# amirkdv/biseqt

Hardware: AMD Instinct MI355X
Metric: GCUPS (DP cell updates/s) banded local align (higher is better)
Workload: dtype i16

## Files before the change

### biseqt_amd/csrc/pw_wave.h

```cpp
#ifndef PW_WAVE_H
#define PW_WAVE_H

#ifndef PW_FN
#error "PW_FN must be defined by the includer"
#endif

#include "pw_types.h"

namespace pw {

template <typename T> struct ScoreTraits;
template <> struct ScoreTraits<int32_t> {
  static constexpr bool is_int = true;
  PW_FN static int32_t neg() { return -(1 << 28); }
  PW_FN static int32_t zero_blk() { return 0; }
  PW_FN static int32_t max2(int32_t a, int32_t b) { return a > b ? a : b; }
  PW_FN static int32_t gap_offer(bool kept, int32_t go, int32_t A) { return kept ? A : A + go; }
};
template <> struct ScoreTraits<double> {
  static constexpr bool is_int = false;
  PW_FN static double neg() { return -1.0e300; }
  PW_FN static double zero_blk() { return -0.0; }
  PW_FN static double max2(double a, double b) { return __builtin_fmax(a, b); }
  union D2I_ { double d; int32_t i[2]; };
// ... 273 lines not shown
    const int wo = (xfeed_o + 8 * b) >> 2, wm = (yfeed_m + 8 * b) >> 2;
    fo_n0 = P::const_dword(oseq, pw_clampi(wo, 0, owlast)); fo_n1 = P::const_dword(oseq, pw_clampi(wo + 1, 0, owlast));
    fo_n2 = P::const_dword(oseq, pw_clampi(wo + 2, 0, owlast));
    fm_n0 = P::const_dword(mseq, pw_clampi(wm, 0, mwlast)); fm_n1 = P::const_dword(mseq, pw_clampi(wm + 1, 0, mwlast));
    fm_n2 = P::const_dword(mseq, pw_clampi(wm + 2, 0, mwlast));
  }
  PW_FN void feed_commit(int b) {
    const int ro = (xfeed_o + 8 * b) & 3, rm = (yfeed_m + 8 * b) & 3;
    fo_lo = funnel(fo_n1, fo_n0, ro); fo_hi = funnel(fo_n2, fo_n1, ro);
    fm_lo = funnel(fm_n1, fm_n0, rm); fm_hi = funnel(fm_n2, fm_n1, rm);
  }

  template <bool RAMP>
  PW_FN void block(int b) {
    if (RAMP) {
#pragma unroll 1
      for (int k = 0; k < 8; k++) iteration<true>(8 * b + k, k);
    } else {
#pragma unroll
      for (int k = 0; k < 8; k++) iteration<false>(8 * b + k, k);
    }
  }

  PW_FN void store_masks(int b) {
    if (lane >= 0 && lane * BK < ndiag && P::central()) {
      uint32_t* dst = a.masks + pd.mask_off;
#pragma unroll
      for (int j = 0; j < BK; j++) dst[mask_word_index(BK, pd.nl, b, lane, j)] = m[j];
    }
  }

  PW_FN void init(int it0 = 0) {
    lane = P::lane();
    X = pd.X; Y = pd.Y; ndiag = pd.ndiag;
    oseq = a.arena + pd.o_off; mseq = a.arena + pd.m_off;
    olast = X > 0 ? X - 1 : 0; mlast = Y > 0 ? Y - 1 : 0;
    owlast = olast >> 2; mwlast = mlast >> 2;
    njl = lane < 0 ? 0 : ndiag - lane * BK;
    uin_next = Tr::neg();
    const int e = (pd.s0 + pd.dmin) >> 1;
    const int f = (pd.s0 - pd.dmin) >> 1;
    xbase = e + it0 + lane * R;
    ybase = f + it0 - lane * R;
    xfeed_o = e + P::nlanes() * R - 1;
    yfeed_m = f - P::lane0() * R;
#pragma unroll
    for (int j = 0; j < BK; j++) {
      H[j] = Tr::neg(); U[j] = Tr::neg(); L[j] = Tr::neg();
      best[j] = Tr::neg(); bestT[j] = 0; m[j] = 0;
      blkL[j] = (lane * BK + j == ndiag) ? Tr::neg() : Tr::zero_blk();
    }
#pragma unroll
    for (int i = 0; i < R; i++) {
      ow[i] = (uint32_t)oseq[pw_clampi(xbase + i - 1, 0, olast)] * osc();
      mw[i] = (uint32_t)mseq[pw_clampi(ybase - i - 1, 0, mlast)] * msc();
    }
    if (AHEAD) {
#pragma unroll
      for (int i = 0; i < (AHEAD ? R : 1); i++) sE[i] = subst(ow[i], mw[i]);
    }
  }

  PW_FN void run() {
    init();
    feed_issue(0);
    for (int b = 0; b < pd.nblocks; b++) {
      feed_commit(b);
      if (b + 1 < pd.nblocks) feed_issue(b + 1);
      if (b >= pd.steady_b0 && b < pd.steady_b1) block<false>(b);
      else block<true>(b);
      store_masks(b);
    }
    finish();
  }

  PW_FN void run_tile() {
    const int bb0 = a.tile_b0, bb1 = a.tile_b0 + a.tile_nb, pitch = a.st_pitch;
    lane = P::lane();
    ndiag = pd.ndiag;
    int w4[4] = {-0x7fffffff, -0x7fffffff, -0x7fffffff, -0x7fffffff};
#pragma unroll
    for (int j = 0; j < BK; j++) {
      const int dd = lane * BK + j;
      if (lane >= 0 && dd < ndiag) {
        const int d = pd.dmin + dd;
        const int tf = (d < 0 ? -d : d) - pd.s0;
        const int tl = tf + 2 * ((d > 0 ? 0 : d) + (pd.X - d > pd.Y ? pd.Y : pd.X - d));
        w4[0] = -tf > w4[0] ? -tf : w4[0]; w4[1] = tf > w4[1] ? tf : w4[1];
        w4[2] = -tl > w4[2] ? -tl : w4[2]; w4[3] = tl > w4[3] ? tl : w4[3];
      }
    }
    P::wg_max4(w4);
    const int tfmin = -w4[0], tfmax = w4[1], tlmin = -w4[2], tlmax = w4[3];
    int bA = tfmin >> 4, bB = tlmax >> 4;
    if (w4[1] == -0x7fffffff) { bA = 1; bB = 0; }
    bA = bA < bb0 ? bb0 : bA; bB = bB > bb1 - 1 ? bb1 - 1 : bB;
    if (bA > bB) {
      if (P::central()) {
#pragma unroll
        for (int j = 0; j < BK; j++) {
          const int dd = lane * BK + j;
          if (lane >= 0 && dd < ndiag) {
#pragma unroll
            for (int r = 0; r < 5; r++)
              a.st_out[r * pitch + dd] = bb0 > 0 ? a.st_in[r * pitch + dd] : (r == 4 ? T(0) : Tr::neg());
          }
        }
      }
      return;
    }
    init(8 * bA);
    if (bb0 > 0) {
#pragma unroll
      for (int j = 0; j < BK; j++) {
        const int dd = lane * BK + j;
        if (lane >= 0 && dd < ndiag) {
          H[j] = a.st_in[dd]; U[j] = a.st_in[pitch + dd]; L[j] = a.st_in[2 * pitch + dd];
          best[j] = a.st_in[3 * pitch + dd]; bestT[j] = (int32_t)a.st_in[4 * pitch + dd];
        }
      }
      uint32_t none = 0;
      uin_next = U[BK - 1];
      xshift_pair<P, false>(uin_next, Tr::neg(), none, 0u, 1);
    }
    feed_issue(bA);
    for (int b = bA; b <= bB; b++) {
      feed_commit(b);
      if (b < bB) feed_issue(b + 1);
      if (16 * b > tfmax && 16 * b + 15 <= tlmin) block<false>(b);
      else block<true>(b);
      store_masks(b);
    }
    if (P::central()) {
#pragma unroll
      for (int j = 0; j < BK; j++) {
        const int dd = lane * BK + j;
        if (lane >= 0 && dd < ndiag) {
          a.st_out[dd] = H[j]; a.st_out[pitch + dd] = U[j]; a.st_out[2 * pitch + dd] = L[j];
          a.st_out[3 * pitch + dd] = best[j]; a.st_out[4 * pitch + dd] = (T)bestT[j];
        }
      }
    }
  }

  PW_FN void finish() {
    const int endrule = a.endrule;
    T cs = Tr::neg(); uint64_t ck = ~(uint64_t)0; int cx = -1, cy = -1; bool have = false;
#pragma unroll
    for (int j = 0; j < BK; j++) {
      const int dd = lane * BK + j;
      const int d = pd.dmin + dd;
      const bool inband = dd < ndiag;
      const bool ends_right = d < X - Y;
      const int lx = ends_right ? d + Y : X, ly = ends_right ? Y : X - d;
      T s; uint64_t k; int x, y; bool ok = inband;
      if (endrule == END_CORNER) {
        ok = ok && (d == X - Y); s = H[j]; k = 0; x = X; y = Y;
      } else if (endrule == END_STD_OVERLAP) {
        s = H[j]; x = lx; y = ly; k = ends_right ? (uint64_t)(uint32_t)lx : (uint64_t)(uint32_t)(X + ly);
      } else if (endrule == END_BANDED_OVERLAP) {
        s = H[j]; x = lx; y = ly; k = (uint64_t)(uint32_t)dd;
      } else {
        const int tfirst = (d < 0 ? -d : d) - pd.s0;
        const int aa = (bestT[j] - tfirst) >> 1;
        s = best[j]; x = aa + (d > 0 ? d : 0); y = aa - (d < 0 ? d : 0);
        if (endrule == END_STD_LOCAL) k = (uint64_t)(uint32_t)x * (uint64_t)(uint32_t)(Y + 1) + (uint64_t)(uint32_t)y;
        else k = ((uint64_t)(uint32_t)dd << 32) | (uint64_t)(uint32_t)aa;
      }
      const bool better = ok && (!have || s > cs || (s == cs && k < ck));
      if (better) { cs = s; ck = k; cx = x; cy = y; have = true; }
    }
    int hv = have ? 1 : 0;
#pragma unroll
    for (int off = 32; off >= 1; off >>= 1) {
      const T os = xshfl_xor<P>(cs, off);
      const uint64_t ok_ = xshfl_xor<P>(ck, off);
      const int ox = P::shfl_xor(cx, off), oy = P::shfl_xor(cy, off), oh = P::shfl_xor(hv, off);
      const bool take = oh && (!hv || os > cs || (os == cs && ok_ < ck));
      if (take) { cs = os; ck = ok_; cx = ox; cy = oy; hv = 1; }
    }
    if (P::nwaves() > 1) {
      T bs = cs; uint64_t bk_ = ck; int bx = cx, by = cy, bh = 0;
      for (int wv = 0; wv < P::nwaves(); wv++) {
        const T os = xwave_bcast<P>(cs, wv);
        const uint64_t ok_ = xwave_bcast<P>(ck, wv);
        const int ox = P::wave_bcast(cx, wv), oy = P::wave_bcast(cy, wv), oh = P::wave_bcast(hv, wv);
        const bool take = oh && (!bh || os > bs || (os == bs && ok_ < bk_));
        if (take) { bs = os; bk_ = ok_; bx = ox; by = oy; bh = 1; }
      }
      cs = bs; ck = bk_; cx = bx; cy = by; hv = bh;
    }
    if (lane == 0) {
      Result r;
      r.score = (double)cs * a.score_mul;
      r.opt_i = a.banded ? cx - cy - pd.dmin : cx;
      r.opt_j = a.banded ? (cx < cy ? cx : cy) : cy;
      r.origin_idx = 0; r.mutant_idx = 0; r.tx_len = 0; r.status = 0;
      if (!hv || (endrule == END_STD_LOCAL && !(cs > T(0)))) { r.opt_i = -1; r.opt_j = -1; r.score = 0.0; }
      a.results[pair_slot] = r;
    }
  }
  int pair_slot;
};

struct __attribute__((aligned(8))) U4 { uint32_t x, y, z, w; };
struct __attribute__((packed)) PackedU64 { uint64_t v; };
struct __attribute__((packed)) PackedU32 { uint32_t v; };

namespace pk {
#if defined(__HIP_DEVICE_COMPILE__)
typedef short s2_t __attribute__((ext_vector_type(2)));
typedef unsigned short u2_t __attribute__((ext_vector_type(2)));
PW_FN s2_t as_s2(uint32_t v) { return __builtin_bit_cast(s2_t, v); }
PW_FN u2_t as_u2(uint32_t v) { return __builtin_bit_cast(u2_t, v); }
PW_FN uint32_t add(uint32_t a, uint32_t b) { return __builtin_bit_cast(uint32_t, (u2_t)(as_u2(a) + as_u2(b))); }
PW_FN uint32_t sub(uint32_t a, uint32_t b) { return __builtin_bit_cast(uint32_t, (u2_t)(as_u2(a) - as_u2(b))); }
PW_FN uint32_t subsat(uint32_t a, uint32_t b) { return __builtin_bit_cast(uint32_t, __builtin_elementwise_sub_sat(as_u2(a), as_u2(b))); }
PW_FN uint32_t max(uint32_t a, uint32_t b) { return __builtin_bit_cast(uint32_t, __builtin_elementwise_max(as_s2(a), as_s2(b))); }
PW_FN uint32_t minu(uint32_t a, uint32_t b) { return __builtin_bit_cast(uint32_t, __builtin_elementwise_min(as_u2(a), as_u2(b))); }
PW_FN uint32_t maxu(uint32_t a, uint32_t b) { return __builtin_bit_cast(uint32_t, __builtin_elementwise_max(as_u2(a), as_u2(b))); }
PW_FN uint32_t shru(uint32_t a, uint32_t sh) { return __builtin_bit_cast(uint32_t, (u2_t)(as_u2(a) >> as_u2(sh))); }
PW_FN uint32_t mad(uint32_t a, uint32_t b, uint32_t c) { return __builtin_bit_cast(uint32_t, (u2_t)(as_u2(a) * as_u2(b) + as_u2(c))); }
PW_FN uint32_t mins(uint32_t a, uint32_t b) { return __builtin_bit_cast(uint32_t, __builtin_elementwise_min(as_s2(a), as_s2(b))); }
PW_FN uint32_t align16(uint32_t hi, uint32_t lo) { return __builtin_amdgcn_alignbit(hi, lo, 16); }
PW_FN uint32_t sign(uint32_t a, uint32_t sh15) { return __builtin_bit_cast(uint32_t, (s2_t)(as_s2(a) >> as_s2(sh15))); }
PW_FN uint32_t opaque(uint32_t v) { asm volatile("" : "+v"(v)); return v; }
PW_FN uint32_t opaque_su(uint32_t v) { asm volatile("" : "+s"(v)); return v; }
PW_FN uint8_t* opaque_s(uint8_t* v) { asm volatile("" : "+s"(v)); return v; }
PW_FN void store_global(uint8_t* base, uint32_t off, const U4& v) {
  typedef __attribute__((address_space(1))) uint8_t gbyte_t;
  typedef __attribute__((address_space(1))) U4 gu4_t;
  *(gu4_t*)((gbyte_t*)base + off) = v;
}
PW_FN uint32_t perm(uint32_t a, uint32_t b, uint32_t sel) { return __builtin_amdgcn_perm(a, b, sel); }
#else
PW_FN uint32_t mk(uint32_t lo, uint32_t hi) { return (lo & 0xffffu) | (hi << 16); }
PW_FN int32_t sl(uint32_t v) { return (int16_t)(v & 0xffffu); }
PW_FN int32_t sh(uint32_t v) { return (int16_t)(v >> 16); }
PW_FN uint32_t add(uint32_t a, uint32_t b) { return mk((a & 0xffffu) + (b & 0xffffu), (a >> 16) + (b >> 16)); }
PW_FN uint32_t sub(uint32_t a, uint32_t b) { return mk((a & 0xffffu) - (b & 0xffffu), (a >> 16) - (b >> 16)); }
PW_FN uint32_t subsat(uint32_t a, uint32_t b) {
  const uint32_t al = a & 0xffffu, bl = b & 0xffffu, ah = a >> 16, bh = b >> 16;
  return mk(al > bl ? al - bl : 0u, ah > bh ? ah - bh : 0u);
}
PW_FN uint32_t max(uint32_t a, uint32_t b) { return mk((uint32_t)(sl(a) > sl(b) ? sl(a) : sl(b)), (uint32_t)(sh(a) > sh(b) ? sh(a) : sh(b))); }
PW_FN uint32_t minu(uint32_t a, uint32_t b) {
  const uint32_t al = a & 0xffffu, bl = b & 0xffffu, ah = a >> 16, bh = b >> 16;
  return mk(al < bl ? al : bl, ah < bh ? ah : bh);
}
PW_FN uint32_t mad(uint32_t a, uint32_t b, uint32_t c) {
  return mk((uint32_t)(sl(a) * sl(b) + sl(c)), (uint32_t)(sh(a) * sh(b) + sh(c)));
}
PW_FN uint32_t maxu(uint32_t a, uint32_t b) {
  const uint32_t al = a & 0xffffu, bl = b & 0xffffu, ah = a >> 16, bh = b >> 16;
  return mk(al > bl ? al : bl, ah > bh ? ah : bh);
}
PW_FN uint32_t shru(uint32_t a, uint32_t sh) { return mk((a & 0xffffu) >> (sh & 0xfu), (a >> 16) >> ((sh >> 16) & 0xfu)); }
PW_FN uint32_t mins(uint32_t a, uint32_t b) { return mk((uint32_t)(sl(a) < sl(b) ? sl(a) : sl(b)), (uint32_t)(sh(a) < sh(b) ? sh(a) : sh(b))); }
PW_FN uint32_t align16(uint32_t hi, uint32_t lo) { return (lo >> 16) | (hi << 16); }
PW_FN uint32_t sign(uint32_t a, uint32_t) { return mk(sl(a) < 0 ? 0xffffu : 0u, sh(a) < 0 ? 0xffffu : 0u); }
PW_FN uint32_t opaque(uint32_t v) { return v; }
PW_FN uint32_t opaque_su(uint32_t v) { return v; }
PW_FN uint8_t* opaque_s(uint8_t* v) { return v; }
PW_FN void store_global(uint8_t* base, uint32_t off, const U4& v) { *(U4*)(base + off) = v; }
PW_FN uint32_t perm(uint32_t a, uint32_t b, uint32_t sel) {
  const uint64_t in = ((uint64_t)a << 32) | b;
  uint32_t r = 0;
  for (int i = 0; i < 4; i++) {
    const uint32_t c = (sel >> (8 * i)) & 0xffu;
    uint32_t v;
    if (c >= 13) v = 0xffu;
    else if (c == 12) v = 0u;
    else if (c >= 8) v = ((in >> (8 * (2 * (c - 8) + 1) + 7)) & 1u) ? 0xffu : 0u;
    else v = (uint32_t)(in >> (8 * c)) & 0xffu;
    r |= v << (8 * i);
  }
  return r;
}
#endif
PW_FN uint32_t both(int32_t v) { return ((uint32_t)v & 0xffffu) | ((uint32_t)v << 16); }
PW_FN uint32_t pack(int32_t lo, int32_t hi) { return ((uint32_t)lo & 0xffffu) | ((uint32_t)hi << 16); }
PW_FN int32_t lo_s(uint32_t v) { return (int32_t)(int16_t)(v & 0xffffu); }
PW_FN int32_t hi_s(uint32_t v) { return (int32_t)(int16_t)(v >> 16); }
}

template <class P, int BK, bool SEG, int RULE = 0, bool MAT = false>
struct WaveFill16 {
  static constexpr bool SC4 = RULE == 3;
  static constexpr int RL = SC4 ? 0 : RULE;
  static constexpr int SCL = SC4 ? 4 : 1;
  static constexpr bool ANYB = RL == 0 || RL == 4;
  static constexpr bool TRK = RL == 0 || RL == 5;
  static constexpr bool CAP = !TRK;
  static_assert(BK % 4 == 0, "packed layout needs an even number of cells per step");
  static constexpr int R = BK / 2;
  static constexpr int RH = R / 2;
#ifdef PW_FILL16_UNR
  static constexpr int UNR = PW_FILL16_UNR;
#else
  static constexpr int UNR = BK <= 8 ? 4 : (BK <= 16 ? 2 : 1);
#endif
  static constexpr int32_t NEG16 = ANYB ? -8192 : -24000;
  static constexpr uint32_t SENT_O = 0xfffeu, SENT_M = 0xffffu;
  static constexpr uint32_t MSEL = 0x0c00u, MSENT_LO = 0x0c08u, MSENT_HI = 0x0c0cu;
  using Base = WaveFill<P, int32_t, BK, true, true, false>;

  const FillParams<int32_t>& a;
  const WaveDesc wd;
  PairDesc pd;
  int li;
  bool valid, segfirst, seglast;
  int pair_slot;
  const uint8_t* oseq;
  const uint8_t* mseq;
  int X, Y, ndiag, owlast, mwlast, xfeed_o, yfeed_m;
  uint32_t fo_lo, fo_hi, fm_lo, fm_hi, fo_n0, fo_n1, fo_n2, fm_n0, fm_n1, fm_n2;

  uint32_t HE[RH], UE[RH], LE[RH], HO[RH], UO[RH], LO[RH];
  uint32_t bestE[RH], bestO[RH], btE[RH], btO[RH];
  uint32_t gebE[RH], gebO[RH];
  uint32_t clE[RH], clO[RH];
  uint32_t tfE[RH], tfO[RH], tlE[RH], tlO[RH];
  uint32_t accE[RH], accO[RH], acc2E[RH], acc2O[RH];
  uint32_t OW[RH], MW[RH];
  uint32_t ROW[MAT ? R : 1];
  uint32_t BIASV, MADJ;
  uint32_t MR0, MR1, MR2, MR3;
  uint32_t ONE, SH15, C2, C4, C16, NDELTA, MATCHV, GOV, GOVI, NEGV, LIMV;
  uint32_t kbE[RH], kbO[RH], C8, SEVEN;
  uint32_t up_prev;
  uint32_t left_next;
  int phase_l, phase_r;
  uint32_t mrow0, mrow_step, mspare, mgroup;
  static constexpr bool SPLIT = ANYB && MAT;
  static constexpr bool SBASE = !SEG && SPLIT;
  uint32_t mrowb;
  uint8_t* mbase[BK / 4];

  PW_FN WaveFill16(const FillParams<int32_t>& a_, const WaveDesc& wd_) : a(a_), wd(wd_) {}

  template <int EK>
  PW_FN void cellpair(uint32_t& Hs, uint32_t& Us, uint32_t& Ls, uint32_t& bests, uint32_t& bts, uint32_t geb,
                      uint32_t tf, uint32_t tl, uint32_t& acc, uint32_t up, uint32_t left, uint32_t oc,
                      uint32_t mc, uint32_t tv, uint32_t clampL = 0, uint32_t och = 0) {
    constexpr bool EDGE = EK != 0;
    uint32_t hM;
    constexpr bool FLOOR0 = MAT && ANYB && (EK & 1) == 0;
    if (MAT) {
      const uint32_t hb = pk::add(Hs, pk::perm(och, oc, mc));
      hM = FLOOR0 ? pk::subsat(hb, BIASV) : pk::sub(hb, BIASV);
    } else {
      const uint32_t ne = pk::minu(oc ^ mc, ONE);
      hM = pk::add(Hs, pk::mad(ne, NDELTA, MATCHV));
    }
    uint32_t Hn = pk::max(pk::max(up, left), hM);
    uint32_t nB;
    if (ANYB) {
      if (EK & 1) Hn = pk::max(Hn, pk::sign(pk::sub(tv, tf), SH15) & NEGV);
      else if (!FLOOR0) Hn = pk::max(Hn, 0u);
      nB = pk::minu(Hn, ONE);
    } else {
      const uint32_t Bc = EDGE ? pk::mad(pk::minu(tv ^ tf, ONE), NEGV, 0u) : NEGV;
      Hn = pk::max(Hn, Bc);
      nB = pk::minu(Hn ^ Bc, ONE);
    }
    const uint32_t nD = pk::minu(Hn ^ up, SC4 ? C2 : ONE);
    const uint32_t nI = pk::minu(Hn ^ left, SC4 ? C4 : ONE);
    const uint32_t hg = pk::add(Hn, geb);
    Us = pk::mad(nD, GOV, hg);
    Ls = pk::mad(nI, GOVI, hg);
    if (!ANYB) Ls = pk::mins(Ls, clampL);
    if (SC4) acc = pk::mad(acc, C16, nB + nD + nI);
    else acc = pk::mad(acc, C16, pk::mad(nI, C4, pk::mad(nD, C2, nB)));
    if (TRK) {
    } else if (EK & 2) {
      const uint32_t e = pk::minu(tv ^ tl, ONE);
      bests = pk::mad(e, pk::sub(bests, Hn), Hn);
    }
    Hs = Hn;
  }

  PW_FN void stamp_best(uint32_t& bts, uint32_t kb, uint32_t kb0, uint32_t blk8) {
    const uint32_t ch = pk::minu((kb ^ kb0) & ~SEVEN, ONE);
    bts = pk::maxu(bts, pk::mad(ch, blk8, kb & SEVEN));
  }

  template <int EK>
  PW_FN void track_key(uint32_t& kb, uint32_t H, uint32_t tl, uint32_t tv, int k) {
    const uint32_t hk = (!ANYB || (EK & 1)) ? pk::max(H, 0u) : H;
    uint32_t key = pk::mad(hk, SC4 ? C2 : C8, pk::both(7 - k));
    if (EK & 2) key &= ~pk::sign(pk::sub(tl, tv), SH15);
    kb = pk::maxu(kb, key);
  }

  template <int EK, int HALF>
  PW_FN void iteration16(int it, int k) {
    constexpr bool EDGE = EK != 0;
    const uint32_t tv0 = pk::both(2 * it), tv1 = pk::both(2 * it + 1);
    {
      uint32_t prev = up_prev;
      if (SEG) prev = segfirst ? NEGV : prev;
      const uint32_t up0 = pk::align16(UO[RH - 1], prev);
#pragma unroll
      for (int p = 0; p < RH; p++)
      {
        cellpair<EK>(HE[p], UE[p], LE[p], bestE[p], btE[p], gebE[p], tfE[p], tlE[p], HALF == 0 ? accE[p] : acc2E[p],
                     p == 0 ? up0 : UO[p == 0 ? 0 : p - 1], LO[p], MAT ? ROW[MAT ? p : 0] : OW[p], MW[p], tv0, clE[p],
                     MAT ? ROW[MAT ? p + RH : 0] : 0u);
        if (TRK) track_key<EK>(kbE[p], HE[p], tlE[p], tv0, k);
      }
    }
    {
      const int oi = xfeed_o + it;
      const uint32_t fb = Base::feed_byte(fo_lo, fo_hi, k);
      uint32_t feed = (!EDGE || (uint32_t)oi < (uint32_t)X) ? fb : SENT_O;
      if (MAT) feed = row_of(fb);
      int32_t mv[2] = {(int32_t)(MAT ? ROW[0] : OW[0]), (int32_t)LE[0]};
      const int32_t mo[2] = {(int32_t)feed, (int32_t)left_next};
      xshlv<P, 2>(mv, mo, phase_l); phase_l ^= 1;
      uint32_t nxt = (uint32_t)mv[0];
      left_next = (uint32_t)mv[1];
      if (SEG) nxt = seglast ? feed : nxt;
      if (MAT) {
#pragma unroll
        for (int i = 0; i + 1 < (MAT ? R : 1); i++) ROW[i] = ROW[i + 1];
        ROW[MAT ? R - 1 : 0] = nxt;
      } else {
        const uint32_t last = pk::align16(nxt, OW[0]);
#pragma unroll
        for (int p = 0; p + 1 < RH; p++) OW[p] = OW[p + 1];
        OW[RH - 1] = last;
      }
    }
    {
      uint32_t nxt = left_next;
      if (SEG) nxt = seglast ? NEGV : nxt;
      const uint32_t leftl = pk::align16(nxt, LE[0]);
#pragma unroll
      for (int p = 0; p < RH; p++)
      {
        cellpair<EK>(HO[p], UO[p], LO[p], bestO[p], btO[p], gebO[p], tfO[p], tlO[p], HALF == 0 ? accO[p] : acc2O[p],
                     UE[p], p == RH - 1 ? leftl : LE[p == RH - 1 ? p : p + 1], MAT ? ROW[MAT ? p : 0] : OW[p], MW[p], tv1, clO[p],
                     MAT ? ROW[MAT ? p + RH : 0] : 0u);
        if (TRK) track_key<EK>(kbO[p], HO[p], tlO[p], tv1, k);
      }
    }
    {
      const int mi = yfeed_m + it;
      const uint32_t fbm = Base::feed_byte(fm_lo, fm_hi, k);
      const uint32_t feed = (MAT ? (MSEL | (fbm + 4u))
                                 : ((!EDGE || (uint32_t)mi < (uint32_t)Y) ? fbm : SENT_M)) << 16;
      int32_t mv[2] = {(int32_t)MW[RH - 1], (int32_t)UO[RH - 1]};
      const int32_t mo[2] = {(int32_t)feed, (int32_t)up_prev};
      xshrv<P, 2>(mv, mo, phase_r); phase_r ^= 1;
      uint32_t prv = (uint32_t)mv[0];
      up_prev = (uint32_t)mv[1];
      if (SEG) prv = segfirst ? feed : prv;
      uint32_t first = pk::align16(MW[RH - 1], prv);
      if (MAT) first += MADJ;
#pragma unroll
      for (int p = RH - 1; p > 0; p--) MW[p] = MW[p - 1];
      MW[0] = first;
    }
  }

  template <int EK>
  PW_FN void block16(int b) {
#pragma unroll
    for (int p = 0; p < RH; p++) { accE[p] = 0; accO[p] = 0; acc2E[p] = 0; acc2O[p] = 0; }
    uint32_t kb0E[RH], kb0O[RH];
    if (TRK) {
#pragma unroll
      for (int p = 0; p < RH; p++) { kb0E[p] = kbE[p]; kb0O[p] = kbO[p]; }
    }
#pragma clang loop unroll_count(UNR)
    for (int k = 0; k < 4; k++) iteration16<EK, 0>(8 * b + k, k);
#pragma clang loop unroll_count(UNR)
    for (int k = 4; k < 8; k++) iteration16<EK, 1>(8 * b + k, k);
    if (TRK) {
      const uint32_t blk8 = pk::both(8 * b + 8);
#pragma unroll
      for (int p = 0; p < RH; p++) {
        stamp_best(btE[p], kbE[p], kb0E[p], blk8);
        stamp_best(btO[p], kbO[p], kb0O[p], blk8);
      }
    }
    {
      uint32_t mwd[BK];
#pragma unroll
      for (int p = 0; p < RH; p++) {
        const uint32_t kE = 0x77777777u - accE[p], k2E = 0x77777777u - acc2E[p];
        const uint32_t kO = 0x77777777u - accO[p], k2O = 0x77777777u - acc2O[p];
        mwd[2 * p] = pk::perm(kE, k2E, 0x05040100u);
        mwd[2 * p + R] = pk::perm(kE, k2E, 0x07060302u);
        mwd[2 * p + 1] = pk::perm(kO, k2O, 0x05040100u);
        mwd[2 * p + 1 + R] = pk::perm(kO, k2O, 0x07060302u);
      }
      if (!SBASE) {
        const uint32_t row = b < pd.nblocks ? mrow0 + (uint32_t)b * mrow_step : mspare;
        uint32_t* dst = a.masks + pd.mask_off;
#pragma unroll
        for (int g = 0; g < BK / 4; g++) {
          U4 v; v.x = mwd[4 * g]; v.y = mwd[4 * g + 1]; v.z = mwd[4 * g + 2]; v.w = mwd[4 * g + 3];
          *(U4*)(dst + (row + (uint32_t)g * mgroup)) = v;
        }
      } else {
#pragma unroll
        for (int g = 0; g < BK / 4; g++) {
          U4 v; v.x = mwd[4 * g]; v.y = mwd[4 * g + 1]; v.z = mwd[4 * g + 2]; v.w = mwd[4 * g + 3];
          pk::store_global(mbase[g], mrowb, v);
        }
        mrowb += 4u * mrow_step;
      }
    }
  }

  PW_FN void feed_issue(int b) {
    const uint32_t* o32 = (const uint32_t*)oseq;
    const uint32_t* m32 = (const uint32_t*)mseq;
    const int wo = (xfeed_o + 8 * b) >> 2, wm = (yfeed_m + 8 * b) >> 2;
    if (!SEG) {
      fo_n0 = P::const_dword(oseq, pw_clampi(wo, 0, owlast)); fo_n1 = P::const_dword(oseq, pw_clampi(wo + 1, 0, owlast));
      fo_n2 = P::const_dword(oseq, pw_clampi(wo + 2, 0, owlast));
      fm_n0 = P::const_dword(mseq, pw_clampi(wm, 0, mwlast)); fm_n1 = P::const_dword(mseq, pw_clampi(wm + 1, 0, mwlast));
      fm_n2 = P::const_dword(mseq, pw_clampi(wm + 2, 0, mwlast));
      return;
    }
    fo_n0 = o32[pw_clampi(wo, 0, owlast)]; fo_n1 = o32[pw_clampi(wo + 1, 0, owlast)]; fo_n2 = o32[pw_clampi(wo + 2, 0, owlast)];
    fm_n0 = m32[pw_clampi(wm, 0, mwlast)]; fm_n1 = m32[pw_clampi(wm + 1, 0, mwlast)]; fm_n2 = m32[pw_clampi(wm + 2, 0, mwlast)];
  }
  PW_FN static int clamp08(int v) {
    if (SEG) return pw_clampi(v, 0, 8);
    const int r = (int)pk::opaque_su((uint32_t)(v > 0 ? v : 0));
    return r < 8 ? r : 8;
  }
  PW_FN static uint64_t inside_bytes(int i0, int n) {
    const int lo = clamp08(-i0), hi = clamp08(n - i0);
    const uint64_t below_hi = hi >= 8 ? ~(uint64_t)0 : (((uint64_t)1 << (8 * hi)) - 1);
    const uint64_t below_lo = lo >= 8 ? ~(uint64_t)0 : (((uint64_t)1 << (8 * lo)) - 1);
    return below_hi & ~below_lo;
  }
  PW_FN void feed_commit(int b, bool edge) {
    const int ro = (xfeed_o + 8 * b) & 3, rm = (yfeed_m + 8 * b) & 3;
    fo_lo = Base::funnel(fo_n1, fo_n0, ro); fo_hi = Base::funnel(fo_n2, fo_n1, ro);
    fm_lo = Base::funnel(fm_n1, fm_n0, rm); fm_hi = Base::funnel(fm_n2, fm_n1, rm);
    if (MAT && edge) {
      const uint64_t io = inside_bytes(xfeed_o + 8 * b, X), im = inside_bytes(yfeed_m + 8 * b, Y);
      const uint64_t o = ((((uint64_t)fo_hi) << 32) | fo_lo) | ~io;
      const uint64_t m = (((((uint64_t)fm_hi) << 32) | fm_lo) & im) | (0x0808080808080808ull & ~im);
      fo_lo = (uint32_t)o; fo_hi = (uint32_t)(o >> 32);
      fm_lo = (uint32_t)m; fm_hi = (uint32_t)(m >> 32);
      if (!SEG) { fo_hi = pk::opaque_su(fo_hi); fm_hi = pk::opaque_su(fm_hi); }
    }
  }

  PW_FN int tfirst_of(int j) const {
    const int dd = li * BK + j, d = pd.dmin + dd;
    return (valid && dd < ndiag) ? (d < 0 ? -d : d) - pd.s0 : 32767;
  }
  PW_FN int tlast_of(int j) const {
    const int dd = li * BK + j, d = pd.dmin + dd;
    if (!valid || dd >= ndiag) return -1;
    const int len = 1 + (d > 0 ? 0 : d) + (X - d > Y ? Y : X - d);
    return (d < 0 ? -d : d) - pd.s0 + 2 * (len - 1);
  }
  PW_FN int tbegin_of(int j) const {
    const int dd = li * BK + j, d = pd.dmin + dd;
    if (!valid || dd >= ndiag) return 32767;
    if ((RL == 2 || RL == 5 || a.brule == BRULE_ORIGIN) && d != 0) return 32767;
    return (d < 0 ? -d : d) - pd.s0;
  }
  PW_FN uint32_t row_of(uint32_t l) const {
    uint32_t r = l == 3u ? MR3 : 0u;
    r = l == 2u ? MR2 : r;
    r = l == 1u ? MR1 : r;
    return l == 0u ? MR0 : r;
  }
  PW_FN uint32_t row_at(int i) const { return (uint32_t)i < (uint32_t)X ? row_of((uint32_t)oseq[i]) : 0u; }
  PW_FN uint32_t msel_lo(int i) const { return (uint32_t)i < (uint32_t)Y ? (MSEL | (uint32_t)mseq[i]) : MSENT_LO; }
  PW_FN uint32_t msel_hi(int i) const { return (uint32_t)i < (uint32_t)Y ? (MSEL | ((uint32_t)mseq[i] + 4u)) : MSENT_HI; }
  PW_FN uint32_t letter_o(int i) const { return (uint32_t)i < (uint32_t)X ? (uint32_t)oseq[i] : SENT_O; }
  PW_FN uint32_t letter_m(int i) const { return (uint32_t)i < (uint32_t)Y ? (uint32_t)mseq[i] : SENT_M; }
  PW_FN int blocked(int j) const { return li * BK + j == ndiag ? NEG16 : 0; }

  PW_FN void run() {
    const int lane = P::lane();
    const int nl = wd.nl;
    const int seg = lane / nl;
    li = lane - seg * nl;
    valid = seg < wd.count;
    segfirst = li == 0; seglast = li == nl - 1;
    const int slot = wd.first + ((SEG && valid) ? seg : 0);
    pair_slot = a.order ? a.order[slot] : slot;
    if (!SEG) pair_slot = P::uniform(pair_slot);
    pd = a.pairs[pair_slot];
    X = pd.X; Y = pd.Y; ndiag = pd.ndiag;
    oseq = a.arena + pd.o_off; mseq = a.arena + pd.m_off;
    owlast = (X > 0 ? X - 1 : 0) >> 2; mwlast = (Y > 0 ? Y - 1 : 0) >> 2;
    const int e = (pd.s0 + pd.dmin) >> 1;
    const int f = (pd.s0 - pd.dmin) >> 1;
    const int xbase = e + li * R, ybase = f - li * R;
    xfeed_o = e + nl * R - 1;
    yfeed_m = f;
    ONE = pk::opaque(0x00010001u); SH15 = pk::opaque(0x000f000fu);
    C2 = pk::opaque(0x00020002u); C4 = pk::opaque(0x00040004u); C16 = pk::opaque(0x00100010u);
    C8 = pk::opaque(0x00080008u); SEVEN = pk::opaque(0x00070007u);
    NEGV = pk::both(NEG16); LIMV = pk::both(-32767);
    NDELTA = pk::both(SCL * (a.mismatch - a.match)); MATCHV = pk::both(SCL * a.match);
    GOV = pk::both(SC4 ? 2 * a.go : a.go); GOVI = pk::both(a.go);
    BIASV = pk::both(a.mat_bias); MADJ = 0x0003fffcu;
    MR0 = a.mat_rows[0]; MR1 = a.mat_rows[1]; MR2 = a.mat_rows[2]; MR3 = a.mat_rows[3];
    if (MAT) {
#pragma unroll
      for (int i = 0; i < (MAT ? R : 1); i++) ROW[i] = row_at(xbase + i - 1);
    }
#pragma unroll
    for (int p = 0; p < RH; p++) {
      const int e0 = 2 * p, e1 = 2 * p + R, o0 = 2 * p + 1, o1 = 2 * p + 1 + R;
      if (ANYB) {
        gebE[p] = pk::pack(SCL * a.ge + blocked(e0), SCL * a.ge + blocked(e1));
        gebO[p] = pk::pack(SCL * a.ge + blocked(o0), SCL * a.ge + blocked(o1));
        tfE[p] = pk::pack(tfirst_of(e0), tfirst_of(e1)); tfO[p] = pk::pack(tfirst_of(o0), tfirst_of(o1));
        clE[p] = clO[p] = 0;
      } else {
        gebE[p] = gebO[p] = pk::both(a.ge);
        clE[p] = pk::pack(blocked(e0) ? NEG16 : 32767, blocked(e1) ? NEG16 : 32767);
        clO[p] = pk::pack(blocked(o0) ? NEG16 : 32767, blocked(o1) ? NEG16 : 32767);
        tfE[p] = pk::pack(tbegin_of(e0), tbegin_of(e1)); tfO[p] = pk::pack(tbegin_of(o0), tbegin_of(o1));
      }
      tlE[p] = pk::pack(tlast_of(e0), tlast_of(e1)); tlO[p] = pk::pack(tlast_of(o0), tlast_of(o1));
      HE[p] = UE[p] = LE[p] = HO[p] = UO[p] = LO[p] = NEGV;
      up_prev = left_next = NEGV; phase_l = 0; phase_r = 0;
      bestE[p] = bestO[p] = NEGV;
      kbE[p] = kbO[p] = 0u; btE[p] = btO[p] = 0u;
      OW[p] = pk::pack((int32_t)letter_o(xbase + p - 1), (int32_t)letter_o(xbase + p + RH - 1));
      if (MAT) MW[p] = pk::pack((int32_t)msel_lo(ybase - p - 1), (int32_t)msel_hi(ybase - p - RH - 1));
      else MW[p] = pk::pack((int32_t)letter_m(ybase - p - 1), (int32_t)letter_m(ybase - p - RH - 1));
    }
    const int sb1 = CAP ? wd.steady_b1 - 1 : wd.steady_b1;
    mgroup = 4u * (uint32_t)pd.nl;
    mspare = (uint32_t)mask_word_index(BK, pd.nl, pd.nblocks, 0, 0);
    const bool mrow_ok = valid && li < pd.nl;
    mrow0 = mrow_ok ? (uint32_t)mask_word_index(BK, pd.nl, 0, li, 0) : mspare;
    mrow_step = mrow_ok ? (uint32_t)mask_word_index(BK, pd.nl, 1, 0, 0) : 0u;
    mrowb = 4u * mrow0;
    if (SBASE) {
#pragma unroll
      for (int g = 0; g < BK / 4; g++)
        mbase[g] = pk::opaque_s((uint8_t*)(a.masks + pd.mask_off) + (uint64_t)(4u * (uint32_t)g * mgroup));
    }
    feed_issue(0);
    if constexpr (SPLIT) {
      const int nb = nblocks_run();
      const int b0 = wd.steady_b0 < nb ? (wd.steady_b0 > 0 ? wd.steady_b0 : 0) : nb;
      const int b1 = sb1 < nb ? sb1 : nb;
      int b = 0;
      if (sb1 > wd.steady_b0) for (; b < b0; b++) blocks_step<1>(b);
      else for (; b < b0; b++) blocks_step<3>(b);
      for (; b < b1; b++) blocks_step<0>(b);
      for (; b < nb; b++) blocks_step<2>(b);
    } else {
      for (int b = 0, nb = nblocks_run(); b < nb; b++) {
        const bool steady = b >= wd.steady_b0 && b < sb1;
        feed_commit(b, !steady);
        if (b + 1 < nb) feed_issue(b + 1);
        if (steady) block16<0>(b);
        else if (!ANYB) block16<3>(b);
        else if (b >= wd.steady_b0) block16<2>(b);
        else if (sb1 > wd.steady_b0) block16<1>(b);
        else block16<3>(b);
      }
    }
    finish();
  }
  PW_FN int nblocks_run() const { return SBASE ? (wd.nblocks < pd.nblocks ? wd.nblocks : pd.nblocks) : wd.nblocks; }
  template <int EK>
  PW_FN void blocks_step(int b) {
    feed_commit(b, EK != 0);
    if (b + 1 < nblocks_run()) feed_issue(b + 1);
    block16<EK>(b);
  }

  PW_FN void finish() {
    const int endrule = a.endrule;
    int32_t cs = -32768; uint64_t ck = ~(uint64_t)0; int cx = -1, cy = -1; bool have = false;
    uint32_t parked[4 * RH];
#pragma unroll
    for (int p = 0; p < RH; p++) {
      parked[4 * p] = TRK ? pk::opaque(kbE[p]) : bestE[p]; parked[4 * p + 1] = TRK ? pk::opaque(btE[p]) : 0u;
      parked[4 * p + 2] = TRK ? pk::opaque(kbO[p]) : bestO[p]; parked[4 * p + 3] = TRK ? pk::opaque(btO[p]) : 0u;
    }
#pragma unroll 1
    for (int q = 0; q < 2 * RH; q++) {
      const int p = q >> 1, odd = q & 1;
      const uint32_t bq = parked[4 * p + 2 * odd], tq = parked[4 * p + 2 * odd + 1];
#pragma unroll 1
      for (int h = 0; h < 2; h++) {
        const int j = 2 * p + odd + h * R;
        const int dd = li * BK + j, d = pd.dmin + dd;
        const int tfirst = (d < 0 ? -d : d) - pd.s0;
        int32_t s; int bt;
        if (TRK) {
          const uint32_t key = h ? (bq >> 16) : (bq & 0xffffu), stamp = h ? (tq >> 16) : (tq & 0xffffu);
          s = (int32_t)(key >> 3);
          if (stamp < 8u) bt = ANYB ? (int)((uint32_t)tfirst & 0xffffu) : 0;
          else bt = 16 * ((int)(stamp >> 3) - 1) + 2 * (7 - (int)(stamp & 7u)) + odd;
        } else {
          s = (h ? pk::hi_s(bq) : pk::lo_s(bq)) / SCL;
          bt = 0;
        }
        const int aa = (bt - tfirst) >> 1;
        int x = aa + (d > 0 ? d : 0), y = aa - (d < 0 ? d : 0);
        uint64_t k;
        bool ok = true;
        if (CAP) {
          const bool ends_right = d < X - Y;
          x = ends_right ? d + Y : X; y = ends_right ? Y : X - d;
          k = endrule == END_STD_OVERLAP ? (uint64_t)(uint32_t)(x < X ? x : X + y) : (uint64_t)(uint32_t)dd;
          if (RL == 2 || RL == 4 || endrule == END_CORNER) ok = d == X - Y;
        } else if (endrule == END_STD_LOCAL) k = (uint64_t)(uint32_t)x * (uint64_t)(uint32_t)(Y + 1) + (uint64_t)(uint32_t)y;
        else k = ((uint64_t)(uint32_t)dd << 32) | (uint64_t)(uint32_t)aa;
        const bool better = ok && valid && dd < ndiag && (!have || s > cs || (s == cs && k < ck));
        if (better) { cs = s; ck = k; cx = x; cy = y; have = true; }
      }
    }
    const int lane = P::lane();
    const int seg = lane / wd.nl;
    for (int sidx = 0; sidx < wd.count; sidx++) {
      int hv = (have && seg == sidx) ? 1 : 0;
      int32_t rs = cs; uint64_t rk = ck; int rx = cx, ry = cy;
#pragma unroll
      for (int off = 32; off >= 1; off >>= 1) {
        const int32_t os = P::shfl_xor(rs, off);
        const uint64_t ok_ = xshfl_xor<P>(rk, off);
        const int ox = P::shfl_xor(rx, off), oy = P::shfl_xor(ry, off), oh = P::shfl_xor(hv, off);
        const bool take = oh && (!hv || os > rs || (os == rs && ok_ < rk));
        if (take) { rs = os; rk = ok_; rx = ox; ry = oy; hv = 1; }
      }
      if (P::nwaves() > 1) {
        int32_t bs = rs; uint64_t bk_ = rk; int bx = rx, by = ry, bh = 0;
        for (int wv = 0; wv < P::nwaves(); wv++) {
          const int32_t os = P::wave_bcast(rs, wv);
          const uint64_t ok_ = xwave_bcast<P>(rk, wv);
          const int ox = P::wave_bcast(rx, wv), oy = P::wave_bcast(ry, wv), oh = P::wave_bcast(hv, wv);
          const bool take = oh && (!bh || os > bs || (os == bs && ok_ < bk_));
          if (take) { bs = os; bk_ = ok_; bx = ox; by = oy; bh = 1; }
        }
        rs = bs; rk = bk_; rx = bx; ry = by; hv = bh;
      }
      if (seg == sidx && li == 0) {
        Result r;
        r.score = (double)rs * a.score_mul;
        r.opt_i = a.banded ? rx - ry - pd.dmin : rx;
        r.opt_j = a.banded ? (rx < ry ? rx : ry) : ry;
        r.origin_idx = 0; r.mutant_idx = 0; r.tx_len = 0; r.status = 0;
        if (!hv || (endrule == END_STD_LOCAL && !(rs > 0))) { r.opt_i = -1; r.opt_j = -1; r.score = 0.0; }
        a.results[pair_slot] = r;
      }
    }
  }
};

PW_FN int pw_first_op(uint32_t mask) {
  return (mask & 1u) ? 0 : (mask & 2u) ? 1 : (mask & 4u) ? 2 : 3;
}


enum { WIN_B = 4, WIN_WORDS = WIN_B * 2 * 4 };

PW_FN void trace_walk(const TraceParams& p, int pair, uint32_t* win ) {
  const PairDesc pdv = p.pairs[pair];
  if (!pdv.solvable || pdv.layout != 0) return;
  Result r = p.results[pair];
  const int ei = p.ends ? p.ends[2 * pair] : r.opt_i;
  const int ej = p.ends ? p.ends[2 * pair + 1] : r.opt_j;
  if (ei < 0 || ej < 0) { r.tx_len = 0; r.status = 0; p.results[pair] = r; return; }
  const int dmin = pdv.dmin, s0 = pdv.s0, ndiag = pdv.ndiag, bk = pdv.bk, nl = pdv.nl, gosign = p.gosign;
  int x = ei, y = ej;
  if (p.banded) {
    const int d = ei + dmin;
    x = ej + (d > 0 ? d : 0); y = ej - (d > 0 ? 0 : d);
  }
  const uint32_t* __restrict__ plane = p.masks + pdv.mask_off;
  uint8_t* __restrict__ tx = p.transcripts + pdv.tx_off;
  const int lgG = bk < 4 ? 1 : 2;
  const int G = 1 << lgG;
  const int njg = bk >> lgG;
  const int ngroups = (ndiag + G - 1) >> lgG;
  int pos = pdv.tx_cap;
  int nms = 0, bad = 0;
  int prev = 3;
  bool done = false;
  while (!done) {
    const int dd0 = x - y - dmin, t0 = x + y - s0;
    if (x < 0 || y < 0 || x > pdv.X || y > pdv.Y || dd0 < 0 || dd0 >= ndiag) { bad = 1; break; }
    const int cb = t0 >> 4;
    const int ga = dd0 >> lgG;
    int gb = ((dd0 & (G - 1)) >= (G >> 1)) ? ga + 1 : ga - 1;
    gb = gb < 0 ? ga + 1 : (gb >= ngroups ? ga - 1 : gb);
    if (gb < 0) gb = ga;
#pragma unroll
    for (int s2 = 0; s2 < 2; s2++) {
      const int gg = s2 ? gb : ga;
      const int ln = gg / njg, jg = gg - ln * njg;
#pragma unroll
      for (int k = 0; k < WIN_B; k++) {
        const int bb = cb - k > 0 ? cb - k : 0;
        const U4 v = *(const U4*)(plane + ((uint64_t)((uint64_t)bb * njg + jg) * nl + ln) * G);
        uint32_t* wslot = win + (k * 2 + s2) * 4;
        wslot[0] = v.x; wslot[1] = v.y; wslot[2] = v.z; wslot[3] = v.w;
      }
    }
    while (true) {
      const int dd = x - y - dmin, t = x + y - s0;
      if (x < 0 || y < 0 || x > pdv.X || y > pdv.Y || dd < 0 || dd >= ndiag) { bad = 1; done = true; break; }
      const int gg = dd >> lgG, b = t >> 4, kb = cb - b;
      if ((gg != ga && gg != gb) || kb < 0 || kb >= WIN_B) break;
      const uint32_t w = win[(kb * 2 + (gg == ga ? 0 : 1)) * 4 + (dd & (G - 1))];
      const uint32_t pm = (w >> (4 * (7 - ((t & 15) >> 1)))) & 15u;
      int op;
      if (prev == 3 || gosign == 0) op = pw_first_op(pm);
      else if (gosign < 0) op = (pm & (1u << prev)) ? prev : pw_first_op(pm);
      else { const uint32_t others = pm & ~(1u << prev); op = others ? pw_first_op(others) : prev; }
      if (op == 0 || pos <= 0) { done = true; break; }
      tx[--pos] = op == 3 ? 'X' : (op == 1 ? 'D' : 'I');
      nms += (op == 3);
      x -= (op != 2); y -= (op != 1);
      prev = op;
      if (op == 3) {
        const int n = ((t & 15) >> 1) - 1;
        if (n >= 0 && pos >= 16) {
          const uint64_t v = (uint64_t)((w & 0x77777777u) >> (4 * (7 - n))) | ((uint64_t)1 << (4 * (n + 1)));
          int k = (int)(__builtin_ctzll(v) >> 2);
          const int lim = x < y ? x : y;
          k = k < lim ? k : lim;
          if (k > 0) {
            PackedU64 xs; xs.v = 0x5858585858585858ull;
            *(PackedU64*)(tx + pos - 8) = xs;
            pos -= k; nms += k; x -= k; y -= k;
          }
        }
      }
    }
  }
  r.origin_idx = x; r.mutant_idx = y;
  r.tx_len = pdv.tx_cap - pos;
  r.status = ST_TRACED | (r.tx_len == 0 ? ST_EMPTY : 0) | ((x + y + nms <= 0) ? ST_PANICK : 0) | (bad ? ST_BADPATH : 0);
  p.results[pair] = r;
}

PW_FN void trace_fixup_serial(const TraceParams& p, int pair) {
  const PairDesc& pd = p.pairs[pair];
  if (!pd.solvable) return;
  const Result r = p.results[pair];
  if (!(r.status & ST_TRACED) || r.tx_len <= 0) return;
  const uint8_t* oseq = p.arena + pd.o_off;
  const uint8_t* mseq = p.arena + pd.m_off;
  uint8_t* tx = p.transcripts + pd.tx_off + pd.tx_cap - r.tx_len;
  int x = r.origin_idx, y = r.mutant_idx;
  for (int k = 0; k < r.tx_len; k++) {
    const uint8_t ch = tx[k];
    if (ch == 'X') { tx[k] = (oseq[x] == mseq[y]) ? 'M' : 'S'; x++; y++; }
    else if (ch == 'D') x++;
    else y++;
  }
}

}
#endif
```

Baseline: 2613.

## Fix selector parity for RH=2 matrix path and invert traceback flags

```diff
diff --git a/biseqt_amd/csrc/pw_wave.h b/biseqt_amd/csrc/pw_wave.h
--- a/biseqt_amd/csrc/pw_wave.h
+++ b/biseqt_amd/csrc/pw_wave.h
@@ -599,7 +599,10 @@
 #endif
   static constexpr int32_t NEG16 = ANYB ? -8192 : -24000;
   static constexpr uint32_t SENT_O = 0xfffeu, SENT_M = 0xffffu;
-  static constexpr uint32_t MSEL = 0x0c00u, MSENT_LO = 0x0c08u, MSENT_HI = 0x0c0cu;
+  static constexpr uint32_t MSEL = 0x0c00u, MOUT = 8u;
+  static constexpr bool FIXSEL = MAT && RH == 2;
+  PW_FN static uint32_t sel4_fed(int it) { return ((uint32_t)it >> 1) & 1u; }
+  PW_FN static bool sel4_lo(int k, int p) { return (((k + 7 - p) >> 1) & 1) != 0; }
   using Base = WaveFill<P, int32_t, BK, true, true, false>;
 
   const FillParams<int32_t>& a;
@@ -630,6 +633,7 @@
   int phase_l, phase_r;
   uint32_t mrow0, mrow_step, mspare, mgroup;
   static constexpr bool SPLIT = ANYB && MAT;
+  static constexpr bool KEPT = SC4 && SPLIT;
   static constexpr bool SBASE = !SEG && SPLIT;
   uint32_t mrowb;
   uint8_t* mbase[BK / 4];
@@ -639,12 +643,12 @@
   template <int EK>
   PW_FN void cellpair(uint32_t& Hs, uint32_t& Us, uint32_t& Ls, uint32_t& bests, uint32_t& bts, uint32_t geb,
                       uint32_t tf, uint32_t tl, uint32_t& acc, uint32_t up, uint32_t left, uint32_t oc,
-                      uint32_t mc, uint32_t tv, uint32_t clampL = 0, uint32_t och = 0) {
+                      uint32_t mc, uint32_t tv, uint32_t clampL = 0, uint32_t och = 0, bool lo4 = false) {
     constexpr bool EDGE = EK != 0;
     uint32_t hM;
     constexpr bool FLOOR0 = MAT && ANYB && (EK & 1) == 0;
     if (MAT) {
-      const uint32_t hb = pk::add(Hs, pk::perm(och, oc, mc));
+      const uint32_t hb = pk::add(Hs, lo4 ? pk::perm(oc, och, mc) : pk::perm(och, oc, mc));
       hM = FLOOR0 ? pk::subsat(hb, BIASV) : pk::sub(hb, BIASV);
     } else {
       const uint32_t ne = pk::minu(oc ^ mc, ONE);
@@ -655,14 +659,14 @@
     if (ANYB) {
       if (EK & 1) Hn = pk::max(Hn, pk::sign(pk::sub(tv, tf), SH15) & NEGV);
       else if (!FLOOR0) Hn = pk::max(Hn, 0u);
-      nB = pk::minu(Hn, ONE);
+      nB = KEPT ? pk::subsat(ONE, Hn) : pk::minu(Hn, ONE);
     } else {
       const uint32_t Bc = EDGE ? pk::mad(pk::minu(tv ^ tf, ONE), NEGV, 0u) : NEGV;
       Hn = pk::max(Hn, Bc);
       nB = pk::minu(Hn ^ Bc, ONE);
     }
-    const uint32_t nD = pk::minu(Hn ^ up, SC4 ? C2 : ONE);
-    const uint32_t nI = pk::minu(Hn ^ left, SC4 ? C4 : ONE);
+    const uint32_t nD = KEPT ? pk::subsat(C2, Hn ^ up) : pk::minu(Hn ^ up, SC4 ? C2 : ONE);
+    const uint32_t nI = KEPT ? pk::subsat(C4, Hn ^ left) : pk::minu(Hn ^ left, SC4 ? C4 : ONE);
     const uint32_t hg = pk::add(Hn, geb);
     Us = pk::mad(nD, GOV, hg);
     Ls = pk::mad(nI, GOVI, hg);
@@ -703,7 +707,7 @@
       {
         cellpair<EK>(HE[p], UE[p], LE[p], bestE[p], btE[p], gebE[p], tfE[p], tlE[p], HALF == 0 ? accE[p] : acc2E[p],
                      p == 0 ? up0 : UO[p == 0 ? 0 : p - 1], LO[p], MAT ? ROW[MAT ? p : 0] : OW[p], MW[p], tv0, clE[p],
-                     MAT ? ROW[MAT ? p + RH : 0] : 0u);
+                     MAT ? ROW[MAT ? p + RH : 0] : 0u, FIXSEL && sel4_lo(k, p));
         if (TRK) track_key<EK>(kbE[p], HE[p], tlE[p], tv0, k);
       }
     }
@@ -738,14 +742,14 @@
       {
         cellpair<EK>(HO[p], UO[p], LO[p], bestO[p], btO[p], gebO[p], tfO[p], tlO[p], HALF == 0 ? accO[p] : acc2O[p],
                      UE[p], p == RH - 1 ? leftl : LE[p == RH - 1 ? p : p + 1], MAT ? ROW[MAT ? p : 0] : OW[p], MW[p], tv1, clO[p],
-                     MAT ? ROW[MAT ? p + RH : 0] : 0u);
+                     MAT ? ROW[MAT ? p + RH : 0] : 0u, FIXSEL && sel4_lo(k, p));
         if (TRK) track_key<EK>(kbO[p], HO[p], tlO[p], tv1, k);
       }
     }
     {
       const int mi = yfeed_m + it;
       const uint32_t fbm = Base::feed_byte(fm_lo, fm_hi, k);
-      const uint32_t feed = (MAT ? (MSEL | (fbm + 4u))
+      const uint32_t feed = (MAT ? (MSEL | (fbm + 4u * (FIXSEL ? sel4_fed(k) : 1u)))
                                  : ((!EDGE || (uint32_t)mi < (uint32_t)Y) ? fbm : SENT_M)) << 16;
       int32_t mv[2] = {(int32_t)MW[RH - 1], (int32_t)UO[RH - 1]};
       const int32_t mo[2] = {(int32_t)feed, (int32_t)up_prev};
@@ -754,7 +758,7 @@
       up_prev = (uint32_t)mv[1];
       if (SEG) prv = segfirst ? feed : prv;
       uint32_t first = pk::align16(MW[RH - 1], prv);
-      if (MAT) first += MADJ;
+      if (MAT && !FIXSEL) first += MADJ;
 #pragma unroll
       for (int p = RH - 1; p > 0; p--) MW[p] = MW[p - 1];
       MW[0] = first;
@@ -786,8 +790,9 @@
       uint32_t mwd[BK];
 #pragma unroll
       for (int p = 0; p < RH; p++) {
-        const uint32_t kE = 0x77777777u - accE[p], k2E = 0x77777777u - acc2E[p];
-        const uint32_t kO = 0x77777777u - accO[p], k2O = 0x77777777u - acc2O[p];
+        const uint32_t inv = KEPT ? 0u : 0x77777777u;
+        const uint32_t kE = KEPT ? accE[p] : inv - accE[p], k2E = KEPT ? acc2E[p] : inv - acc2E[p];
+        const uint32_t kO = KEPT ? accO[p] : inv - accO[p], k2O = KEPT ? acc2O[p] : inv - acc2O[p];
         mwd[2 * p] = pk::perm(kE, k2E, 0x05040100u);
         mwd[2 * p + R] = pk::perm(kE, k2E, 0x07060302u);
         mwd[2 * p + 1] = pk::perm(kO, k2O, 0x05040100u);
@@ -844,7 +849,7 @@
     if (MAT && edge) {
       const uint64_t io = inside_bytes(xfeed_o + 8 * b, X), im = inside_bytes(yfeed_m + 8 * b, Y);
       const uint64_t o = ((((uint64_t)fo_hi) << 32) | fo_lo) | ~io;
-      const uint64_t m = (((((uint64_t)fm_hi) << 32) | fm_lo) & im) | (0x0808080808080808ull & ~im);
+      const uint64_t m = (((((uint64_t)fm_hi) << 32) | fm_lo) & im) | ((0x0101010101010101ull * MOUT) & ~im);
       fo_lo = (uint32_t)o; fo_hi = (uint32_t)(o >> 32);
       fm_lo = (uint32_t)m; fm_hi = (uint32_t)(m >> 32);
       if (!SEG) { fo_hi = pk::opaque_su(fo_hi); fm_hi = pk::opaque_su(fm_hi); }
@@ -874,8 +879,7 @@
     return l == 0u ? MR0 : r;
   }
   PW_FN uint32_t row_at(int i) const { return (uint32_t)i < (uint32_t)X ? row_of((uint32_t)oseq[i]) : 0u; }
-  PW_FN uint32_t msel_lo(int i) const { return (uint32_t)i < (uint32_t)Y ? (MSEL | (uint32_t)mseq[i]) : MSENT_LO; }
-  PW_FN uint32_t msel_hi(int i) const { return (uint32_t)i < (uint32_t)Y ? (MSEL | ((uint32_t)mseq[i] + 4u)) : MSENT_HI; }
+  PW_FN uint32_t msel(int i, uint32_t plus4) const { return MSEL | (((uint32_t)i < (uint32_t)Y ? (uint32_t)mseq[i] : MOUT) + 4u * plus4); }
   PW_FN uint32_t letter_o(int i) const { return (uint32_t)i < (uint32_t)X ? (uint32_t)oseq[i] : SENT_O; }
   PW_FN uint32_t letter_m(int i) const { return (uint32_t)i < (uint32_t)Y ? (uint32_t)mseq[i] : SENT_M; }
   PW_FN int blocked(int j) const { return li * BK + j == ndiag ? NEG16 : 0; }
@@ -904,7 +908,7 @@
     C8 = pk::opaque(0x00080008u); SEVEN = pk::opaque(0x00070007u);
     NEGV = pk::both(NEG16); LIMV = pk::both(-32767);
     NDELTA = pk::both(SCL * (a.mismatch - a.match)); MATCHV = pk::both(SCL * a.match);
-    GOV = pk::both(SC4 ? 2 * a.go : a.go); GOVI = pk::both(a.go);
+    GOV = pk::both(KEPT ? -2 * a.go : (SC4 ? 2 * a.go : a.go)); GOVI = pk::both(KEPT ? -a.go : a.go);
     BIASV = pk::both(a.mat_bias); MADJ = 0x0003fffcu;
     MR0 = a.mat_rows[0]; MR1 = a.mat_rows[1]; MR2 = a.mat_rows[2]; MR3 = a.mat_rows[3];
     if (MAT) {
@@ -915,8 +919,9 @@
     for (int p = 0; p < RH; p++) {
       const int e0 = 2 * p, e1 = 2 * p + R, o0 = 2 * p + 1, o1 = 2 * p + 1 + R;
       if (ANYB) {
-        gebE[p] = pk::pack(SCL * a.ge + blocked(e0), SCL * a.ge + blocked(e1));
-        gebO[p] = pk::pack(SCL * a.ge + blocked(o0), SCL * a.ge + blocked(o1));
+        const int geo = SCL * a.ge + (KEPT ? SCL * a.go : 0);
+        gebE[p] = pk::pack(geo + blocked(e0), geo + blocked(e1));
+        gebO[p] = pk::pack(geo + blocked(o0), geo + blocked(o1));
         tfE[p] = pk::pack(tfirst_of(e0), tfirst_of(e1)); tfO[p] = pk::pack(tfirst_of(o0), tfirst_of(o1));
         clE[p] = clO[p] = 0;
       } else {
@@ -931,7 +936,10 @@
       bestE[p] = bestO[p] = NEGV;
       kbE[p] = kbO[p] = 0u; btE[p] = btO[p] = 0u;
       OW[p] = pk::pack((int32_t)letter_o(xbase + p - 1), (int32_t)letter_o(xbase + p + RH - 1));
-      if (MAT) MW[p] = pk::pack((int32_t)msel_lo(ybase - p - 1), (int32_t)msel_hi(ybase - p - RH - 1));
+      if (MAT) {
+        const int yl = ybase - p - 1, yh = ybase - p - RH - 1;
+        MW[p] = pk::pack((int32_t)msel(yl, FIXSEL ? sel4_fed(yl - f) : 0u), (int32_t)msel(yh, FIXSEL ? sel4_fed(yh - f) : 1u));
+      }
       else MW[p] = pk::pack((int32_t)letter_m(ybase - p - 1), (int32_t)letter_m(ybase - p - RH - 1));
     }
     const int sb1 = CAP ? wd.steady_b1 - 1 : wd.steady_b1;
```

New measurement: 2699 (median of 6 runs). +3.3%, better.
